# datatypevoid/babble

Measured on AMD Instinct MI355X. Metric: consensus-ordered events/sec at N=256 peers (1 GPU and 8-GPU batched sims), higher is better.
Workload: dtype int32

## Files before the change

### babble_amd/csrc/hgx_cts.hip

```cpp
#include <hip/hip_runtime.h>

#include <algorithm>
#include <climits>
#include <cstdint>

#include "hgx_device.h"
#include "hgx_kernels.h"

namespace hgx {

constexpr int kCpT = 8;
constexpr int kCpRing = 4;
constexpr int kCpMaxC = 4096;
constexpr int64_t kCtsRedo = (int64_t)0x8000000000000000ull;

struct CtsTileInfo {
    int32_t row[kCpT];
    int64_t ts[kCpT];
    int32_t tc, p0;
};

__device__ __forceinline__ void cp_lds_barrier() { asm volatile("s_waitcnt lgkmcnt(0)\n\ts_barrier" ::: "memory"); }
__device__ __forceinline__ void cp_order() { asm volatile("" ::: "memory"); }

template <int NPAD, typename CT>
__global__ void __launch_bounds__(256) k_cts_pipe(const int32_t* __restrict__ fu, const int32_t* __restrict__ rcnt,
                                                  const int32_t* __restrict__ p_rr, const int32_t* __restrict__ c_off,
                                                  const int32_t* __restrict__ c_base, const int32_t* __restrict__ WLAT, const CT* __restrict__ FDT,
                                                  const int64_t* __restrict__ p_ts, int64_t* __restrict__ p_cts, int C,
                                                  int n, int64_t Pcap, int c_lo, int c_cnt, int ntt) {
    constexpr int T = kCpT, LD = T + 1, NG = 256 / T, U = NPAD / NG, CPL = NPAD / 64;
    extern __shared__ __attribute__((aligned(16))) uint8_t dyn[];
    int32_t* kd = (int32_t*)dyn;
    int32_t* tp0 = kd + C;
    int32_t* trc = tp0 + c_cnt;
    uint32_t* vals = (uint32_t*)(dyn + ((4 * (C + 2 * c_cnt) + 15) & ~15));
    uint8_t* memb = (uint8_t*)(vals + 2 * NPAD * LD);
    __shared__ CtsTileInfo ring[kCpRing];
    __shared__ __attribute__((aligned(16))) uint32_t whist[4][256];

    const int t = threadIdx.x;
    for (int c = t; c < C; c += 256) kd[c] = c_off[c] - c_base[c];
    for (int c = t; c < c_cnt; c += 256) {
        tp0[c] = c_off[c_lo + c] + fu[c_lo + c];
        trc[c] = rcnt[c_lo + c];
    }
    __syncthreads();
    const int total = c_cnt * ntt;
    const int gstep = (int)gridDim.x;
    auto next_tile = [&](int u) -> int {
        for (; u < total; u += gstep) {
            const int ci = u % c_cnt, tt = u / c_cnt;
            if (tt * T < trc[ci]) break;
        }
        return __builtin_amdgcn_readfirstlane(min(u, total));
    };
    const int e = t & (T - 1), cg = t / T;
    int32_t l1_rr = -1;
    int64_t l1_ts = 0;
    bool l1_in = false;
    auto l1_issue = [&](int u) {
        const bool vu = u < total;
        const int ci = vu ? u % c_cnt : 0, tt = vu ? u / c_cnt : 0;
        l1_in = vu && tt * T + e < trc[ci];
        const int p = l1_in ? tp0[ci] + tt * T + e : 0;
        l1_rr = p_rr[p];
        l1_ts = p_ts[p];
    };
    auto l1_store = [&](int u, int slot) {
        const bool vu = u < total;
        const int ci = vu ? u % c_cnt : 0, tt = vu ? u / c_cnt : 0;
        int32_t rr_v = l1_in ? l1_rr : -1;
        int64_t ts_v = l1_ts;
        asm volatile("" : "+v"(rr_v), "+v"(ts_v));
        if (t < T) {
            ring[slot].row[t] = rr_v;
            ring[slot].ts[t] = ts_v;
            if (t == 0) {
                ring[slot].tc = c_lo + ci;
                ring[slot].p0 = tp0[ci] + tt * T;
            }
        }
    };
    int32_t l2_w[U];
    CT l2_fd[U];
    auto l2_issue = [&](int slot) {
        const int i = ring[slot].row[e];
        const int tc = ring[slot].tc, g = tc / n;
        const int p = ring[slot].p0 + e;
        const size_t fb = (size_t)max(i, 0) * C + (size_t)g * n;
        const size_t wrow = (fb + (tc - g * n)) * n;
#pragma unroll
        for (int u = 0; u < U; u++) {
            const int c = cg + NG * u;
            const bool in = i >= 0 && c < n;
            const int cc = in ? c : 0;
            l2_w[u] = WLAT[wrow + cc];
            l2_fd[u] = FDT[(size_t)cc * Pcap + (in ? p : 0)];
        }
    };
    int32_t idx[U];
    auto l2_finish = [&](int slot) {
        const int i = ring[slot].row[e];
        const int tc = ring[slot].tc, g = tc / n;
        const int j = ring[slot].p0 + e - kd[tc];
#pragma unroll
        for (int u = 0; u < U; u++) {
            const int c = cg + NG * u;
            const bool in = i >= 0 && c < n;
            const int cc = in ? c : 0;
            const int32_t k = kd[g * n + cc] + Coord<CT>::fd(l2_fd[u]);
            idx[u] = (in & (l2_w[u] >= j)) ? k : -1;
        }
    };

    int u0 = next_tile(blockIdx.x);
    if (u0 >= total) return;
    int u1 = next_tile(u0 + gstep);
    int u2 = next_tile(u1 + gstep);
    l1_issue(u0);
    l1_store(u0, 0);
    l1_issue(u1);
    l1_store(u1, 1);
    __syncthreads();
    l2_issue(0);
    l2_finish(0);
    const int lane = lane_id(), wave = t >> 6;
    int64_t x[U];
#pragma unroll
    for (int u = 0; u < U; u++) x[u] = p_ts[max(idx[u], 0)];
    cp_order();
    l2_issue(1);
    cp_order();
    l1_issue(u2);
    cp_order();

    for (int k = 0; u0 < total; k++) {
        const int s0 = k & (kCpRing - 1), s1 = (k + 1) & (kCpRing - 1), s2 = (k + 2) & (kCpRing - 1);
        {
            uint32_t* v = vals + (k & 1) * NPAD * LD;
            uint8_t* mb = memb + (k & 1) * NPAD * LD;
            const int64_t base = ring[s0].ts[e];
#pragma unroll
            for (int u = 0; u < U; u++) {
                const int c = cg + NG * u;
                const bool ok = idx[u] >= 0;
                const int64_t dlt = x[u] - base;
                const bool ov = ok && (dlt < INT32_MIN || dlt > INT32_MAX);
                v[c * LD + e] = (uint32_t)(int32_t)dlt ^ 0x80000000u;
                mb[c * LD + e] = (uint8_t)((ok ? 1 : 0) | (ov ? 2 : 0));
            }
        }
        l2_finish(s1);
        l1_store(u2, s2);
        cp_lds_barrier();
        const int u3 = next_tile(u2 + gstep);
#pragma unroll
        for (int u = 0; u < U; u++) x[u] = p_ts[max(idx[u], 0)];
        cp_order();
        l2_issue(s2);
        cp_order();
        l1_issue(u3);
        cp_order();
        {
            const uint32_t* v = vals + (k & 1) * NPAD * LD;
            const uint8_t* mb = memb + (k & 1) * NPAD * LD;
            for (int ev = wave; ev < T; ev += 4) {
                if (ring[s0].row[ev] < 0) continue;
                bool ok[CPL];
                uint32_t vv[CPL];
                int m = 0;
                bool any_ov = false;
#pragma unroll
                for (int q = 0; q < CPL; q++) {
                    const int c = lane + 64 * q;
                    const uint8_t b = mb[c * LD + ev];
                    ok[q] = (b & 1) != 0;
                    vv[q] = v[c * LD + ev];
                    m += __popcll(__ballot(ok[q]));
                    any_ov |= __ballot((b & 2) != 0) != 0;
                }
                int64_t res = kCtsRedo;
                if (!any_ov) {
                    const uint32_t sel = wave_select_kth32<CPL>(vv, ok, m / 2, whist[wave]);
                    res = ring[s0].ts[ev] + (int64_t)(int32_t)(sel ^ 0x80000000u);
                }
                if (lane == 0) p_cts[ring[s0].p0 + ev] = res;
            }
        }
        u0 = u1;
        u1 = u2;
        u2 = u3;
    }
}

template <int NPAD, typename CT>
__global__ void __launch_bounds__(256) k_cts_redo(const int32_t* __restrict__ fu, const int32_t* __restrict__ rcnt,
                                                  const int32_t* __restrict__ p_rr, const int32_t* __restrict__ c_off,
                                                  const int32_t* __restrict__ c_base, const int32_t* __restrict__ WLAT,
                                                  const CT* __restrict__ FDT, const int64_t* __restrict__ p_ts,
                                                  int64_t* __restrict__ p_cts, int C, int n, int64_t Pcap, int c_lo) {
    constexpr int CPL = NPAD / 64;
    __shared__ int32_t list[256];
    __shared__ int32_t cnt;
    __shared__ __attribute__((aligned(16))) uint32_t whist[4][256];
    const int gc = c_lo + blockIdx.y, g = gc / n;
    const int k = (int)blockIdx.x * 256 + threadIdx.x;
    if (threadIdx.x == 0) cnt = 0;
    __syncthreads();
    const int64_t p0 = (int64_t)c_off[gc] + fu[gc];
    if (k < rcnt[gc] && p_cts[p0 + k] == kCtsRedo) list[atomicAdd(&cnt, 1)] = k;
    __syncthreads();
    const int lane = lane_id(), wave = threadIdx.x >> 6;
    for (int q0 = wave; q0 < cnt; q0 += 4) {
        const int64_t p = p0 + list[q0];
        const int i = p_rr[p];
        const int j = c_base[gc] + (int)(p - c_off[gc]);
        const size_t row = ((size_t)i * C + gc) * n;
        uint64_t v[CPL];
        bool ok[CPL];
        int m = 0;
#pragma unroll
        for (int q = 0; q < CPL; q++) {
            const int c = lane + 64 * q;
            ok[q] = c < n && WLAT[row + c] >= j;
            int64_t x = 0;
            if (ok[q]) {
                const int ch = g * n + c;
                x = p_ts[c_off[ch] - c_base[ch] + Coord<CT>::fd(FDT[(size_t)c * Pcap + p])];
            }
            v[q] = (uint64_t)x ^ 0x8000000000000000ull;
            m += __popcll(__ballot(ok[q]));
        }
        const int64_t res = (int64_t)(wave_select_kth<CPL>(v, ok, m / 2, whist[wave]) ^ 0x8000000000000000ull);
        if (lane == 0) p_cts[p] = res;
    }
}

template <int NPAD, typename CT>
static bool cts_pipe_launch(hipStream_t s, const DevArrays& a, int c_lo, int c_cnt, int C, int n, int64_t P,
                            int max_cnt) {
    constexpr int LD = kCpT + 1;
    const size_t lds = (((size_t)4 * C + (size_t)8 * c_cnt + 15) & ~(size_t)15) + (size_t)2 * NPAD * LD * 5;
    const void* f = (const void*)k_cts_pipe<NPAD, CT>;
    static int dev_cus[64] = {0};
    int dev = 0;
    if (hipGetDevice(&dev) != hipSuccess || dev < 0 || dev >= 64) return false;
    if (ensure_lds_limit(f, lds) != hipSuccess) return false;
    if (dev_cus[dev] == 0) {
        int cus = 0;
        if (hipDeviceGetAttribute(&cus, hipDeviceAttributeMultiprocessorCount, dev) != hipSuccess || cus <= 0)
            return false;
        dev_cus[dev] = cus;
    }
    int per_cu = 0;
    if (blocks_per_cu(f, 256, lds, &per_cu) != hipSuccess || per_cu < 1) return false;
    const int ntt = (max_cnt + kCpT - 1) / kCpT;
    const int64_t tiles = (int64_t)c_cnt * ntt;
    if (tiles <= 0) return true;
    if (tiles > 0x7FFFFFFF - (int64_t)dev_cus[dev] * per_cu) return false;
    const unsigned grid = (unsigned)std::min<int64_t>(tiles, (int64_t)dev_cus[dev] * per_cu);
    hipLaunchKernelGGL((k_cts_pipe<NPAD, CT>), dim3(grid), dim3(256), lds, s, a.fu, a.rcnt, a.p_rr, a.c_off, a.c_base,
                       a.WLAT, (const CT*)a.FDT, a.p_ts, a.p_cts, C, n, P, c_lo, c_cnt, ntt);
    hipLaunchKernelGGL((k_cts_redo<NPAD, CT>), dim3((max_cnt + 255) / 256, c_cnt), dim3(256), 0, s, a.fu, a.rcnt, a.p_rr,
                       a.c_off, a.c_base, a.WLAT, (const CT*)a.FDT, a.p_ts, a.p_cts, C, n, P, c_lo);
    return true;
}

template <typename CT>
static bool launch_cts_pipe_t(hipStream_t s, const DevArrays& a, int c_lo, int c_cnt, int C, int n, int64_t P,
                              int max_cnt) {
    if (n <= 64) return cts_pipe_launch<64, CT>(s, a, c_lo, c_cnt, C, n, P, max_cnt);
    if (n <= 128) return cts_pipe_launch<128, CT>(s, a, c_lo, c_cnt, C, n, P, max_cnt);
    if (n <= 256) return cts_pipe_launch<256, CT>(s, a, c_lo, c_cnt, C, n, P, max_cnt);
    return cts_pipe_launch<512, CT>(s, a, c_lo, c_cnt, C, n, P, max_cnt);
}

bool cts_pipe_ok(int n, int C) { return n > 32 && n <= 512 && C <= kCpMaxC; }

bool launch_cts_pipe(hipStream_t s, const DevArrays& a, int c_lo, int c_cnt, int C, int n, int64_t P, int max_cnt) {
    if (max_cnt <= 0 || c_cnt <= 0) return true;
    if (!cts_pipe_ok(n, C)) return false;
    return a.compact ? launch_cts_pipe_t<uint16_t>(s, a, c_lo, c_cnt, C, n, P, max_cnt)
                     : launch_cts_pipe_t<int32_t>(s, a, c_lo, c_cnt, C, n, P, max_cnt);
}

constexpr int kRowKMax = 8;
constexpr int kRowTP = 64;
constexpr int kRowD = 16;
constexpr int row_waves(int npad) { return npad >= 128 ? 8 : 4; }

template <int NPAD, typename CT, int TP, int DREQ, int NW>
__global__ void __launch_bounds__(64 * NW) k_cts_row(const int32_t* __restrict__ fu, const int32_t* __restrict__ rcnt,
                                                 const int32_t* __restrict__ p_rr, const int32_t* __restrict__ c_off,
                                                 const int32_t* __restrict__ c_base, const int32_t* __restrict__ WLAT,
                                                 const CT* __restrict__ FDT, const int64_t* __restrict__ p_ts,
                                                 int64_t* __restrict__ p_cts, int C, int n, int64_t Pcap, int c_lo,
                                                 int c_cnt, int R, int K) {
    static_assert(TP == 64, "k_cts_row: a wave's lanes are the block's events");
    constexpr int LD = TP + 1;
    constexpr int CPL = NPAD / 64;
    constexpr int CW = NPAD / NW;
    constexpr int NI = CW;
    constexpr int D = DREQ < NI ? DREQ : NI;
    constexpr int NB = NI / D;
    constexpr int MB = NPAD / 8;
    static_assert(NI % D == 0 && NI % 8 == 0 && NI <= 64, "k_cts_row: batches and membership bytes");
    constexpr int RG = 64 * NW / NPAD;
    constexpr int KL = kRowKMax / RG;
    static_assert(RG >= 1 && kRowKMax % RG == 0, "k_cts_row: staging loads");
    extern __shared__ __attribute__((aligned(16))) uint32_t vals[];
    int32_t* wl = (int32_t*)(vals + NPAD * LD);
    __shared__ uint8_t mem[TP][MB];
    __shared__ int32_t e_row[TP];
    __shared__ int64_t e_ts[TP];
    __shared__ int32_t e_ovf[TP];
    __shared__ uint32_t s_min[NW];
    const int cl = (int)(blockIdx.x % (unsigned)c_cnt), tt = (int)(blockIdx.x / (unsigned)c_cnt);
    const int tc = c_lo + cl;
    const int f0 = fu[tc], co = c_off[tc];
    const int64_t q0 = (int64_t)co + f0, pend = q0 + rcnt[tc];
    const int64_t ps = (int64_t)co + (f0 & ~31) + (int64_t)tt * TP;
    if ((ps > q0 ? ps : q0) >= pend) return;
    const int lane = lane_id(), wave = __builtin_amdgcn_readfirstlane((int)(threadIdx.x >> 6));
    const int e = lane;
    const int64_t p = ps + e;
    const bool ev = p >= q0 && p < pend;
    const int64_t pl = ev ? p : (ps > q0 ? ps : q0);
    const int i = p_rr[pl];
    const int64_t base = p_ts[pl];
    const int g = tc / n, gb = g * n;
    const int j = c_base[tc] + (int)(pl - co);
    const bool evi = ev && i >= 0;
    const int wc0 = wave * CW;
    uint32_t* whist = vals + NPAD * LD + 256 * wave;
    auto chain = [&](int k) { const int c = wc0 + k; return c < n ? c : 0; };
    auto load_fd = [&](int b, CT (&fd)[D]) {
#pragma unroll
        for (int u = 0; u < D; u++) fd[u] = FDT[(size_t)chain(b * D + u) * Pcap + pl];
    };
    CT fd[2][D];
    load_fd(0, fd[0]);
    const int kc = wc0 + lane < n && lane < CW ? wc0 + lane : 0;
    const int32_t kdv = c_off[gb + kc] - c_base[gb + kc];
    const uint32_t wmin = wave_reduce_min_u32(evi ? (uint32_t)i : 0x7fffffffu);
    if (lane == 0) s_min[wave] = wmin;
    if (threadIdx.x < TP) {
        e_row[e] = evi ? i : -1;
        e_ts[e] = base;
        e_ovf[e] = 0;
    }
    cp_lds_barrier();
    uint32_t bmin = s_min[0];
#pragma unroll
    for (int w = 1; w < NW; w++) bmin = min(bmin, s_min[w]);
    const int imin = bmin == 0x7fffffffu ? 0 : (int)bmin;
    int32_t st[KL];
    const int sw = (int)threadIdx.x % NPAD, srow = (int)threadIdx.x / NPAD;
#pragma unroll
    for (int q = 0; q < KL; q++)
        st[q] = WLAT[((size_t)min(imin + min(q * RG + srow, K - 1), R - 1) * C + tc) * n + min(sw, n - 1)];
    int64_t x[2][D];
    auto gather = [&](int b, const CT (&f)[D], int64_t (&xo)[D]) {
#pragma unroll
        for (int u = 0; u < D; u++) {
            const int k = b * D + u;
            const int32_t kd = __builtin_amdgcn_readlane(kdv, k);
            const int32_t fv = Coord<CT>::fd(f[u]);
            xo[u] = p_ts[fv != kMaxI32 ? kd + fv : 0];
        }
    };
    uint64_t ovm = 0;
    if (NB > 1) load_fd(1, fd[1]);
    cp_order();
    gather(0, fd[0], x[0]);
    cp_order();
#pragma unroll
    for (int b = 0; b < NB; b++) {
        if (b + 2 < NB) load_fd(b + 2, fd[b & 1]);
        cp_order();
        if (b + 1 < NB) gather(b + 1, fd[(b + 1) & 1], x[(b + 1) & 1]);
        cp_order();
#pragma unroll
        for (int u = 0; u < D; u++) {
            const int k = b * D + u;
            const int64_t dlt = x[b & 1][u] - base;
            ovm |= (uint64_t)(dlt < INT32_MIN || dlt > INT32_MAX) << k;
            vals[(wc0 + k) * LD + e] = (uint32_t)(int32_t)dlt ^ 0x80000000u;
        }
        cp_order();
    }
    const int WS = n + 1;
#pragma unroll
    for (int q = 0; q < KL; q++)
        if (q * RG + srow < K && sw < n) wl[(q * RG + srow) * WS + sw] = st[q];
    __syncthreads();
    {
        uint64_t okm = 0;
        if (!evi || i - imin < K) {
            const int32_t* row = wl + (evi ? i - imin : 0) * WS;
#pragma unroll
            for (int k = 0; k < NI; k++) okm |= (uint64_t)(row[chain(k)] >= j) << k;
        } else {
            const int32_t* __restrict__ row = WLAT + ((size_t)i * C + tc) * n;
#pragma unroll
            for (int k = 0; k < NI; k++) okm |= (uint64_t)(row[chain(k)] >= j) << k;
        }
        const int live = n - wc0;
        if (live < NI) okm &= live > 0 ? ((uint64_t)1 << live) - 1 : 0;
        if (!evi) okm = 0;
#pragma unroll
        for (int q = 0; q < NI / 8; q++) mem[e][wc0 / 8 + q] = (uint8_t)(okm >> (8 * q));
        if (ovm & okm) e_ovf[e] = 1;
    }
    __syncthreads();
    for (int e2 = wave; e2 < TP; e2 += NW) {
        if (e_row[e2] < 0) continue;
        bool ok[CPL];
        int m = 0;
#pragma unroll
        for (int q = 0; q < CPL; q++) {
            const int c = lane + 64 * q;
            ok[q] = (mem[e2][c >> 3] >> (c & 7)) & 1u;
            m += __popcll(__builtin_amdgcn_ballot_w64(ok[q]));
        }
        int64_t res;
        if (!e_ovf[e2]) {
            uint32_t v[CPL];
#pragma unroll
            for (int q = 0; q < CPL; q++) v[q] = vals[(lane + 64 * q) * LD + e2];
            const uint32_t u = wave_select_kth32_top<CPL>(v, ok, m / 2, whist);
            res = e_ts[e2] + (int64_t)(int32_t)(u ^ 0x80000000u);
        } else {
            uint64_t v[CPL];
#pragma unroll
            for (int q = 0; q < CPL; q++) {
                const int c = lane + 64 * q;
                int64_t x = 0;
                if (ok[q]) x = p_ts[c_off[gb + c] - c_base[gb + c] + Coord<CT>::fd(FDT[(size_t)c * Pcap + ps + e2])];
                v[q] = (uint64_t)x ^ 0x8000000000000000ull;
            }
            res = (int64_t)(wave_select_kth<CPL>(v, ok, m / 2, whist) ^ 0x8000000000000000ull);
        }
        if (lane == 0) p_cts[ps + e2] = res;
    }
}

template <int NPAD, typename CT>
static bool cts_row_launch(hipStream_t s, const DevArrays& a, int c_lo, int c_cnt, int C, int n, int64_t P,
                           int max_cnt, int R, int k_rows) {
    constexpr int TP = kRowTP, NW = row_waves(NPAD);
    constexpr size_t kStatic = (size_t)TP * (NPAD / 8) + (size_t)TP * 16 + 4 * NW;
    const size_t fixed = (size_t)NPAD * (TP + 1) * 4, row = (size_t)(n + 1) * 4;
    const int room = (int)(((size_t)79 * 1024 - kStatic - fixed) / row);
    const int K = k_rows > 0 ? std::min(k_rows, kRowKMax) : std::max(1, std::min(room, kRowKMax));
    const size_t lds = fixed + std::max((size_t)K * row, (size_t)NW * 1024);
    const void* f = (const void*)k_cts_row<NPAD, CT, TP, kRowD, NW>;
    if (ensure_lds_limit(f, lds) != hipSuccess) return false;
    const int64_t blocks = (int64_t)c_cnt * ((max_cnt + 31 + TP - 1) / TP);
    if (blocks > 0x7FFFFFFF) return false;
    hipLaunchKernelGGL((k_cts_row<NPAD, CT, TP, kRowD, NW>), dim3((unsigned)blocks), dim3(64 * NW), lds, s, a.fu, a.rcnt, a.p_rr,
                       a.c_off, a.c_base, a.WLAT, (const CT*)a.FDT, a.p_ts, a.p_cts, C, n, P, c_lo, c_cnt, R, K);
    return true;
}

template <typename CT>
static bool launch_cts_row_t(hipStream_t s, const DevArrays& a, int c_lo, int c_cnt, int C, int n, int64_t P,
                             int max_cnt, int R, int k_rows) {
    if (n <= 64) return cts_row_launch<64, CT>(s, a, c_lo, c_cnt, C, n, P, max_cnt, R, k_rows);
    if (n <= 128) return cts_row_launch<128, CT>(s, a, c_lo, c_cnt, C, n, P, max_cnt, R, k_rows);
    return cts_row_launch<256, CT>(s, a, c_lo, c_cnt, C, n, P, max_cnt, R, k_rows);
}

bool cts_row_ok(int n) { return n > 32 && n <= 256; }
int cts_row_tile() { return kRowTP; }

bool launch_cts_row(hipStream_t s, const DevArrays& a, int c_lo, int c_cnt, int C, int n, int64_t P, int max_cnt,
                    int R, int k_rows) {
    if (max_cnt <= 0 || c_cnt <= 0) return true;
    if (!cts_row_ok(n) || R <= 0) return false;
    return a.compact ? launch_cts_row_t<uint16_t>(s, a, c_lo, c_cnt, C, n, P, max_cnt, R, k_rows)
                     : launch_cts_row_t<int32_t>(s, a, c_lo, c_cnt, C, n, P, max_cnt, R, k_rows);
}

}
```

### babble_amd/csrc/hgx_device.h

```cpp
#pragma once

#include <hip/hip_runtime.h>

#include <cstdint>

namespace hgx {

__device__ __forceinline__ int lane_id() { return (int)(threadIdx.x & 63); }

__device__ __forceinline__ uint32_t block_excl_scan256(uint32_t v, uint32_t* sh, uint32_t* total) {
    const int lane = lane_id(), wave = threadIdx.x >> 6;
    uint32_t x = v;
    for (int o = 1; o < 64; o <<= 1) {
        const uint32_t y = __shfl_up(x, o);
        if (lane >= o) x += y;
    }
    if (lane == 63) sh[wave] = x;
    __syncthreads();
    uint32_t wbase = 0;
    for (int w = 0; w < wave; w++) wbase += sh[w];
    *total = sh[0] + sh[1] + sh[2] + sh[3];
    __syncthreads();
    return wbase + x - v;
}

template <int HD>
__device__ __forceinline__ uint32_t swar_ge_count(const uint32_t (&v)[HD], const uint32_t (&nf)[HD]) {
    uint32_t c = 0;
    if constexpr (HD % 2 == 0) {
#pragma unroll
        for (int i = 0; i < HD / 2; i++) {
            const uint64_t s = ((((uint64_t)v[2 * i + 1]) << 32) | v[2 * i]) + ((((uint64_t)nf[2 * i + 1]) << 32) | nf[2 * i]);
            c = __builtin_popcount((uint32_t)s & 0x80808080u) + c;
            asm volatile("" : "+v"(c));
            c = __builtin_popcount((uint32_t)(s >> 32) & 0x80808080u) + c;
            asm volatile("" : "+v"(c));
        }
    } else {
#pragma unroll
        for (int d = 0; d < HD; d++) c += __builtin_popcount((v[d] + nf[d]) & 0x80808080u);
    }
    return c;
}
__device__ __forceinline__ uint32_t swar_nf(uint32_t fd7) { return 0x80808080u - fd7; }

__device__ __forceinline__ uint64_t group_mask(int gs, int grp) {
    return (gs >= 64) ? ~0ull : (((1ull << gs) - 1ull) << (gs * grp));
}

template <typename CT>
struct Coord;
template <>
struct Coord<int32_t> {
    static constexpr int32_t kLaNone = -1;
    __device__ __forceinline__ static int32_t la(int32_t v) { return v; }
    __device__ __forceinline__ static int32_t enc_la(int32_t v) { return v; }
    __device__ __forceinline__ static int32_t fd(int32_t v) { return v; }
    __device__ __forceinline__ static int32_t enc_fd(int32_t v) { return v; }
};
template <>
struct Coord<uint16_t> {
    static constexpr int32_t kLaNone = 0;
    __device__ __forceinline__ static int32_t la(uint32_t v) { return (int32_t)v - 1; }
    __device__ __forceinline__ static uint16_t enc_la(int32_t v) { return (uint16_t)(v + 1); }
    __device__ __forceinline__ static int32_t fd(uint32_t v) { return v == 0xFFFFu ? 2147483647 : (int32_t)v; }
    __device__ __forceinline__ static uint16_t enc_fd(int32_t v) { return v >= 0xFFFF ? (uint16_t)0xFFFF : (uint16_t)v; }
};

__device__ __forceinline__ void wave_lds_fence() {
    __builtin_amdgcn_fence(__ATOMIC_SEQ_CST, "wavefront");
    __builtin_amdgcn_wave_barrier();
}

__device__ __forceinline__ uint64_t wave_min_u64(uint64_t x) {
    for (int o = 32; o >= 1; o >>= 1) {
        const uint64_t y = __shfl_xor(x, o);
        x = y < x ? y : x;
    }
    return x;
}

__device__ __forceinline__ uint64_t wave_max_u64(uint64_t x) {
    for (int o = 32; o >= 1; o >>= 1) {
        const uint64_t y = __shfl_xor(x, o);
        x = y > x ? y : x;
    }
    return x;
}

template <int CPL>
__device__ uint64_t wave_select_kth(const uint64_t (&v)[CPL], const bool (&ok)[CPL], int K,
                                    uint32_t* __restrict__ hist) {
    const int lane = lane_id();
    uint64_t lo = ~0ull, hi = 0;
#pragma unroll
    for (int q = 0; q < CPL; q++)
        if (ok[q]) { lo = v[q] < lo ? v[q] : lo; hi = v[q] > hi ? v[q] : hi; }
    lo = wave_min_u64(lo);
    hi = wave_max_u64(hi);
    bool act[CPL];
#pragma unroll
    for (int q = 0; q < CPL; q++) act[q] = ok[q];
    uint64_t base = lo;
    uint64_t range = hi - lo;
    int k = K;
    while (range != 0) {
        int bits = 64 - __clzll((long long)range);
        const int shift = bits > 8 ? bits - 8 : 0;
#pragma unroll
        for (int t = 0; t < 4; t++) hist[lane * 4 + t] = 0;
        wave_lds_fence();
#pragma unroll
        for (int q = 0; q < CPL; q++)
            if (act[q]) atomicAdd(&hist[(uint32_t)((v[q] - base) >> shift)], 1u);
        wave_lds_fence();
        uint32_t h[4], s = 0;
#pragma unroll
        for (int t = 0; t < 4; t++) { h[t] = hist[lane * 4 + t]; s += h[t]; }
        uint32_t incl = s;
        for (int o = 1; o < 64; o <<= 1) {
            const uint32_t y = __shfl_up(incl, o);
            if (lane >= o) incl += y;
        }
        const uint32_t excl = incl - s;
        int bucket = -1;
        uint32_t below = 0;
        if ((uint32_t)k >= excl && (uint32_t)k < incl) {
            uint32_t acc = excl;
#pragma unroll
            for (int t = 0; t < 4; t++) {
                if (bucket < 0 && (uint32_t)k < acc + h[t]) { bucket = lane * 4 + t; below = acc; }
                acc += h[t];
            }
        }
        const uint64_t bm = __ballot(bucket >= 0);
        const int src = __ffsll((unsigned long long)bm) - 1;
        bucket = __shfl(bucket, src);
        below = __shfl(below, src);
        wave_lds_fence();
        k -= (int)below;
        const uint64_t nb = base + ((uint64_t)bucket << shift);
#pragma unroll
        for (int q = 0; q < CPL; q++) act[q] = act[q] && ((v[q] - base) >> shift) == (uint64_t)bucket;
        if (shift == 0) return nb;
        const uint64_t top = nb + ((1ull << shift) - 1);
        base = nb;
        range = (top < hi ? top : hi) - nb;
        uint64_t alo = ~0ull, ahi = 0;
#pragma unroll
        for (int q = 0; q < CPL; q++)
            if (act[q]) { alo = v[q] < alo ? v[q] : alo; ahi = v[q] > ahi ? v[q] : ahi; }
        alo = wave_min_u64(alo);
        ahi = wave_max_u64(ahi);
        base = alo;
        range = ahi - alo;
    }
    return base;
}

#define HGX_DPP_SCAN(x, id, OP)                                                                  \
    do {                                                                                         \
        x = OP(x, (uint32_t)__builtin_amdgcn_update_dpp((int)(id), (int)(x), 0x111, 0xf, 0xf, false)); \
        x = OP(x, (uint32_t)__builtin_amdgcn_update_dpp((int)(id), (int)(x), 0x112, 0xf, 0xf, false)); \
        x = OP(x, (uint32_t)__builtin_amdgcn_update_dpp((int)(id), (int)(x), 0x114, 0xf, 0xf, false)); \
        x = OP(x, (uint32_t)__builtin_amdgcn_update_dpp((int)(id), (int)(x), 0x118, 0xf, 0xf, false)); \
        x = OP(x, (uint32_t)__builtin_amdgcn_update_dpp((int)(id), (int)(x), 0x142, 0xa, 0xf, false)); \
        x = OP(x, (uint32_t)__builtin_amdgcn_update_dpp((int)(id), (int)(x), 0x143, 0xc, 0xf, false)); \
    } while (0)
#define HGX_OP_ADD(a, b) ((a) + (b))
#define HGX_OP_MIN(a, b) min((a), (b))
#define HGX_OP_MAX(a, b) max((a), (b))

__device__ __forceinline__ uint32_t wave_scan_add_u32(uint32_t x) { HGX_DPP_SCAN(x, 0u, HGX_OP_ADD); return x; }
__device__ __forceinline__ uint32_t wave_reduce_min_u32(uint32_t x) {
    HGX_DPP_SCAN(x, 0xffffffffu, HGX_OP_MIN);
    return (uint32_t)__builtin_amdgcn_readlane((int)x, 63);
}
__device__ __forceinline__ uint32_t wave_reduce_max_u32(uint32_t x) {
    HGX_DPP_SCAN(x, 0u, HGX_OP_MAX);
    return (uint32_t)__builtin_amdgcn_readlane((int)x, 63);
}

template <int CPL>
__device__ uint32_t wave_select_kth32(const uint32_t (&v)[CPL], const bool (&ok)[CPL], int K,
                                      uint32_t* __restrict__ hist) {
    const int lane = lane_id();
    uint32_t lo = 0xffffffffu, hi = 0;
#pragma unroll
    for (int q = 0; q < CPL; q++)
        if (ok[q]) { lo = min(lo, v[q]); hi = max(hi, v[q]); }
    lo = wave_reduce_min_u32(lo);
    hi = wave_reduce_max_u32(hi);
    const uint32_t range = hi - lo;
    if (range == 0) return lo;
    const int bits = 32 - __clz((int)range);
    uint32_t d[CPL];
    bool act[CPL];
#pragma unroll
    for (int q = 0; q < CPL; q++) { d[q] = v[q] - lo; act[q] = ok[q]; }
    uint4* __restrict__ h4 = (uint4*)hist;
    uint32_t prefix = 0;
    uint32_t k = (uint32_t)K;
    for (int shift = ((bits - 1) / 8) * 8; shift >= 0; shift -= 8) {
        h4[lane] = make_uint4(0u, 0u, 0u, 0u);
        wave_lds_fence();
#pragma unroll
        for (int q = 0; q < CPL; q++)
            if (act[q]) atomicAdd(&hist[(d[q] >> shift) & 255u], 1u);
        wave_lds_fence();
        const uint4 h = h4[lane];
        const uint32_t sum = h.x + h.y + h.z + h.w;
        const uint32_t incl = wave_scan_add_u32(sum);
        const uint32_t excl = incl - sum;
        const uint32_t a1 = excl + h.x, a2 = a1 + h.y, a3 = a2 + h.z;
        const int bt = (k < a1) ? 0 : (k < a2) ? 1 : (k < a3) ? 2 : 3;
        const uint32_t below = (k < a1) ? excl : (k < a2) ? a1 : (k < a3) ? a2 : a3;
        const uint64_t bm = __ballot(k >= excl && k < incl);
        const int src = (int)__builtin_ctzll(bm);
        const uint32_t bucket = (uint32_t)__builtin_amdgcn_readlane(lane * 4 + bt, src);
        k -= (uint32_t)__builtin_amdgcn_readlane((int)below, src);
        wave_lds_fence();
        prefix |= bucket << shift;
#pragma unroll
        for (int q = 0; q < CPL; q++) act[q] = act[q] && ((d[q] >> shift) & 255u) == bucket;
    }
    return lo + prefix;
}

template <int CPL>
__device__ __forceinline__ uint32_t wave_select_kth32_top(const uint32_t (&v)[CPL], const bool (&ok)[CPL], int K,
                                                          uint32_t* __restrict__ hist) {
    constexpr int DB = 6;
    const int lane = lane_id();
    uint32_t lo = 0xffffffffu, hi = 0;
#pragma unroll
    for (int q = 0; q < CPL; q++)
        if (ok[q]) { lo = min(lo, v[q]); hi = max(hi, v[q]); }
    lo = wave_reduce_min_u32(lo);
    hi = wave_reduce_max_u32(hi);
    if (hi <= lo) return lo;
    int top = 32 - __clz((int)(hi - lo));
    uint32_t d[CPL], inc[CPL];
#pragma unroll
    for (int q = 0; q < CPL; q++) { d[q] = v[q] - lo; inc[q] = ok[q] ? 1u : 0u; }
    uint32_t prefix = 0, k = (uint32_t)K;
#pragma unroll 1
    for (int pass = 0; pass < (32 + DB - 1) / DB; pass++) {
        const int shift = top > DB ? top - DB : 0;
        uint32_t dig[CPL];
#pragma unroll
        for (int q = 0; q < CPL; q++) dig[q] = __builtin_amdgcn_ubfe(d[q], (uint32_t)shift, (uint32_t)(top - shift));
        hist[lane] = 0;
        wave_lds_fence();
#pragma unroll
        for (int q = 0; q < CPL; q++) atomicAdd(&hist[dig[q]], inc[q]);
        wave_lds_fence();
        const uint32_t h = hist[lane];
        wave_lds_fence();
        const uint32_t incl = wave_scan_add_u32(h);
        const uint32_t excl = incl - h;
        const uint64_t bm = __builtin_amdgcn_ballot_w64(k >= excl) & __builtin_amdgcn_ballot_w64(k < incl);
        const int bucket = bm ? (int)__builtin_ctzll(bm) : 0;
        k -= (uint32_t)__builtin_amdgcn_readlane((int)excl, bucket);
        const uint32_t cnt = (uint32_t)__builtin_amdgcn_readlane((int)h, bucket);
        prefix |= (uint32_t)bucket << shift;
        if (shift == 0) break;
#pragma unroll
        for (int q = 0; q < CPL; q++) inc[q] = dig[q] == (uint32_t)bucket ? inc[q] : 0u;
        if (cnt == 1u) {
            uint32_t r = lo + prefix;
#pragma unroll
            for (int q = 0; q < CPL; q++) {
                const uint64_t b = __builtin_amdgcn_ballot_w64(inc[q] != 0u);
                if (b) r = (uint32_t)__builtin_amdgcn_readlane((int)v[q], (int)__builtin_ctzll(b));
            }
            return r;
        }
        top = shift;
    }
    return lo + prefix;
}

template <int CPL>
__device__ uint32_t wave_select_kth32_bisect(const uint32_t (&v)[CPL], const bool (&ok)[CPL], int K) {
    uint32_t lo = 0xffffffffu, hi = 0;
#pragma unroll
    for (int q = 0; q < CPL; q++)
        if (ok[q]) { lo = min(lo, v[q]); hi = max(hi, v[q]); }
    lo = wave_reduce_min_u32(lo);
    hi = wave_reduce_max_u32(hi);
    uint32_t a = 0, b = hi - lo;
    uint32_t d[CPL];
#pragma unroll
    for (int q = 0; q < CPL; q++) d[q] = ok[q] ? v[q] - lo : 0xffffffffu;
    while (a < b) {
        const uint32_t mid = a + ((b - a) >> 1);
        int cnt = 0;
#pragma unroll
        for (int q = 0; q < CPL; q++) cnt += __popcll(__ballot(d[q] <= mid));
        if (cnt > K) b = mid;
        else a = mid + 1;
    }
    return lo + a;
}

}
```

Before: 274.8 million.

## Select per-event median with 8-lane groups instead of whole waves

Replaces the per-event whole-wave radix selection with 8-lane DPP groups, so each wave processes 8 events at once. Membership is packed into transposed 32-bit words via LDS atomicOr, and a new group8 radix-select runs its histogram in the event's own column of the vals buffer. Overflow events still fall back to the wave-wide 64-bit selection. The new path adds LDS atomics and more complex control flow, and it restricts NI to at most 32.

```diff
diff --git a/babble_amd/csrc/hgx_cts.hip b/babble_amd/csrc/hgx_cts.hip
--- a/babble_amd/csrc/hgx_cts.hip
+++ b/babble_amd/csrc/hgx_cts.hip
@@ -304,14 +304,14 @@
     constexpr int NI = CW;
     constexpr int D = DREQ < NI ? DREQ : NI;
     constexpr int NB = NI / D;
-    constexpr int MB = NPAD / 8;
-    static_assert(NI % D == 0 && NI % 8 == 0 && NI <= 64, "k_cts_row: batches and membership bytes");
+    constexpr int VPL = NPAD / 8;
+    static_assert(NI % D == 0 && NI % 8 == 0 && NI <= 32 && 8 % NW == 0, "k_cts_row: batches, membership words, groups");
     constexpr int RG = 64 * NW / NPAD;
     constexpr int KL = kRowKMax / RG;
     static_assert(RG >= 1 && kRowKMax % RG == 0, "k_cts_row: staging loads");
     extern __shared__ __attribute__((aligned(16))) uint32_t vals[];
     int32_t* wl = (int32_t*)(vals + NPAD * LD);
-    __shared__ uint8_t mem[TP][MB];
+    __shared__ uint32_t memw[8 * LD];
     __shared__ int32_t e_row[TP];
     __shared__ int64_t e_ts[TP];
     __shared__ int32_t e_ovf[TP];
@@ -350,6 +350,7 @@
         e_ts[e] = base;
         e_ovf[e] = 0;
     }
+    for (int w = (int)threadIdx.x; w < 8 * LD; w += 64 * NW) memw[w] = 0;
     cp_lds_barrier();
     uint32_t bmin = s_min[0];
 #pragma unroll
@@ -409,40 +410,46 @@
         const int live = n - wc0;
         if (live < NI) okm &= live > 0 ? ((uint64_t)1 << live) - 1 : 0;
         if (!evi) okm = 0;
-#pragma unroll
-        for (int q = 0; q < NI / 8; q++) mem[e][wc0 / 8 + q] = (uint8_t)(okm >> (8 * q));
+        const uint32_t ok32 = (uint32_t)okm;
+#pragma unroll
+        for (int l = 0; l < 8; l++)
+            atomicOr(&memw[l * LD + e], ((((ok32 >> l) & 0x01010101u) * 0x10204080u) >> 28) << (wc0 / 8));
         if (ovm & okm) e_ovf[e] = 1;
     }
     __syncthreads();
-    for (int e2 = wave; e2 < TP; e2 += NW) {
-        if (e_row[e2] < 0) continue;
-        bool ok[CPL];
-        int m = 0;
-#pragma unroll
-        for (int q = 0; q < CPL; q++) {
-            const int c = lane + 64 * q;
-            ok[q] = (mem[e2][c >> 3] >> (c & 7)) & 1u;
-            m += __popcll(__builtin_amdgcn_ballot_w64(ok[q]));
-        }
-        int64_t res;
-        if (!e_ovf[e2]) {
-            uint32_t v[CPL];
-#pragma unroll
-            for (int q = 0; q < CPL; q++) v[q] = vals[(lane + 64 * q) * LD + e2];
-            const uint32_t u = wave_select_kth32_top<CPL>(v, ok, m / 2, whist);
-            res = e_ts[e2] + (int64_t)(int32_t)(u ^ 0x80000000u);
-        } else {
+    const int gs = lane >> 3, gl = lane & 7;
+    for (int grp = 0; grp < 8 / NW; grp++) {
+        const int vw = wave + NW * grp, e2 = vw + 8 * gs;
+        const bool has = e_row[e2] >= 0, wide = e_ovf[e2] != 0;
+        if (!__builtin_amdgcn_ballot_w64(has)) continue;
+        const bool part = has && !wide;
+        if (__builtin_amdgcn_ballot_w64(part)) {
+            uint32_t* hcol = vals + e2;
+            const uint32_t member = part ? memw[gl * LD + e2] : 0u;
+            uint32_t v[VPL];
+#pragma unroll
+            for (int q = 0; q < VPL; q++) v[q] = hcol[(gl + 8 * q) * LD];
+            const uint32_t u = group8_select_kth32_top<VPL, LD>(v, member, hcol, whist + 32 * gs, gl);
+            if (part && gl == 0) p_cts[ps + e2] = e_ts[e2] + (int64_t)(int32_t)(u ^ 0x80000000u);
+        }
+        for (uint64_t todo = __builtin_amdgcn_ballot_w64(has && wide) & 0x0101010101010101ull; todo; todo &= todo - 1) {
+            const int e3 = vw + (int)__builtin_ctzll(todo);
+            const uint32_t mw = memw[gl * LD + e3];
+            bool ok[CPL];
             uint64_t v[CPL];
+            int m = 0;
 #pragma unroll
             for (int q = 0; q < CPL; q++) {
                 const int c = lane + 64 * q;
+                ok[q] = (mw >> (gs + 8 * q)) & 1u;
+                m += __popcll(__builtin_amdgcn_ballot_w64(ok[q]));
                 int64_t x = 0;
-                if (ok[q]) x = p_ts[c_off[gb + c] - c_base[gb + c] + Coord<CT>::fd(FDT[(size_t)c * Pcap + ps + e2])];
+                if (ok[q]) x = p_ts[c_off[gb + c] - c_base[gb + c] + Coord<CT>::fd(FDT[(size_t)c * Pcap + ps + e3])];
                 v[q] = (uint64_t)x ^ 0x8000000000000000ull;
             }
-            res = (int64_t)(wave_select_kth<CPL>(v, ok, m / 2, whist) ^ 0x8000000000000000ull);
-        }
-        if (lane == 0) p_cts[ps + e2] = res;
+            const int64_t res = (int64_t)(wave_select_kth<CPL>(v, ok, m / 2, whist) ^ 0x8000000000000000ull);
+            if (lane == 0) p_cts[ps + e3] = res;
+        }
     }
 }
 
@@ -450,7 +457,7 @@
 static bool cts_row_launch(hipStream_t s, const DevArrays& a, int c_lo, int c_cnt, int C, int n, int64_t P,
                            int max_cnt, int R, int k_rows) {
     constexpr int TP = kRowTP, NW = row_waves(NPAD);
-    constexpr size_t kStatic = (size_t)TP * (NPAD / 8) + (size_t)TP * 16 + 4 * NW;
+    constexpr size_t kStatic = (size_t)8 * (TP + 1) * 4 + (size_t)TP * 16 + 4 * NW;
     const size_t fixed = (size_t)NPAD * (TP + 1) * 4, row = (size_t)(n + 1) * 4;
     const int room = (int)(((size_t)79 * 1024 - kStatic - fixed) / row);
     const int K = k_rows > 0 ? std::min(k_rows, kRowKMax) : std::max(1, std::min(room, kRowKMax));
diff --git a/babble_amd/csrc/hgx_device.h b/babble_amd/csrc/hgx_device.h
--- a/babble_amd/csrc/hgx_device.h
+++ b/babble_amd/csrc/hgx_device.h
@@ -281,6 +281,148 @@
     return lo + prefix;
 }
 
+template <int CTRL, int BANK = 0xf>
+__device__ __forceinline__ uint32_t dpp_mov0(uint32_t x) {
+    return (uint32_t)__builtin_amdgcn_update_dpp(0, (int)x, CTRL, 0xf, BANK, false);
+}
+#define HGX_DPP_GROUP8(x, OP)                    \
+    do {                                         \
+        x = OP(x, dpp_mov0<0xB1>(x));            \
+        x = OP(x, dpp_mov0<0x4E>(x));            \
+        x = OP(x, dpp_mov0<0x141>(x));           \
+    } while (0)
+#define HGX_OP_OR(a, b) ((a) | (b))
+__device__ __forceinline__ uint32_t group8_add_u32(uint32_t x) { HGX_DPP_GROUP8(x, HGX_OP_ADD); return x; }
+__device__ __forceinline__ uint32_t group8_or_u32(uint32_t x) { HGX_DPP_GROUP8(x, HGX_OP_OR); return x; }
+__device__ __forceinline__ uint32_t group8_min_u32(uint32_t x) { HGX_DPP_GROUP8(x, HGX_OP_MIN); return x; }
+__device__ __forceinline__ uint32_t group8_max_u32(uint32_t x) { HGX_DPP_GROUP8(x, HGX_OP_MAX); return x; }
+__device__ __forceinline__ uint32_t group8_scan_add_u32(uint32_t x, int l) {
+    const uint32_t y1 = dpp_mov0<0x111>(x);
+    x += l >= 1 ? y1 : 0u;
+    const uint32_t y2 = dpp_mov0<0x112>(x);
+    x += l >= 2 ? y2 : 0u;
+    x += dpp_mov0<0x114, 0xA>(x);
+    return x;
+}
+
+
+struct Group8Sel {
+    uint32_t lo, res, prefix, k;
+    int top;
+    bool live;
+};
+
+template <int NV, int LD>
+__device__ __forceinline__ uint32_t group8_select_pass(const uint32_t (&d)[NV], uint32_t& act, Group8Sel& s,
+                                                       uint32_t* hcol, int l) {
+    constexpr int DB = 6;
+    const int shift = s.top > DB ? s.top - DB : 0;
+    const uint32_t width = (uint32_t)(s.top - shift);
+    auto bin = [&](uint32_t b) -> uint32_t* { return (uint32_t*)((char*)hcol + __umul24(b, (uint32_t)(LD * 4))); };
+#pragma unroll
+    for (int t = 0; t < 8; t++) hcol[(l + 8 * t) * LD] = 0;
+    wave_lds_fence();
+#pragma unroll
+    for (int q = 0; q < NV; q++) atomicAdd(bin(__builtin_amdgcn_ubfe(d[q], (uint32_t)shift, width)), (act >> q) & 1u);
+    wave_lds_fence();
+    uint32_t h[8];
+#pragma unroll
+    for (int t = 0; t < 8; t++) h[t] = hcol[(l + 8 * t) * LD];
+    wave_lds_fence();
+    uint32_t acc = 0, below = 0, hsel = 0, tsel = 0;
+#pragma unroll
+    for (int t = 0; t < 8; t++) {
+        const bool c = s.k >= acc;
+        below = c ? acc : below;
+        hsel = c ? h[t] : hsel;
+        tsel = c ? (uint32_t)t : tsel;
+        acc += group8_add_u32(h[t]);
+    }
+    const uint32_t k1 = s.k - below;
+    const uint32_t incl = group8_scan_add_u32(hsel, l), excl = incl - hsel;
+    const bool own = k1 >= excl && k1 < incl;
+    const uint32_t pk = group8_or_u32(own ? (tsel * 8 + (uint32_t)l) | excl << 6 | hsel << 16 : 0u);
+    const uint32_t bucket = pk & 63u, cnt = pk >> 16;
+    s.k = k1 - ((pk >> 6) & 1023u);
+    s.prefix |= bucket << shift;
+    const bool last = shift == 0, one = cnt == 1u;
+    if (__builtin_amdgcn_ballot_w64(s.live && !last)) {
+        uint32_t keep = 0;
+#pragma unroll
+        for (int q = 0; q < NV; q++) keep |= __builtin_amdgcn_ubfe(d[q], (uint32_t)shift, width) == bucket ? 1u << q : 0u;
+        act &= keep;
+    }
+    if (__builtin_amdgcn_ballot_w64(s.live && !last && one)) {
+        uint32_t w = 0xffffffffu;
+#pragma unroll
+        for (int q = 0; q < NV; q++) w = min(w, d[q] | ~(uint32_t)__builtin_amdgcn_sbfe((int)act, q, 1));
+        w = group8_min_u32(w);
+        s.res = s.live && !last && one ? s.lo + w : s.res;
+    }
+    s.res = s.live && last ? s.lo + s.prefix : s.res;
+    s.live = s.live && !last && !one;
+    act = s.live ? act : 0u;
+    s.top = shift;
+    return cnt;
+}
+
+template <int VPL, int LD>
+__device__ __forceinline__ uint32_t group8_select_kth32_top(uint32_t (&v)[VPL], uint32_t member, uint32_t* hcol,
+                                                            uint32_t* list, int l) {
+    constexpr int DB = 6, PASSES = (32 + DB - 1) / DB, CAP = 32, LV = CAP / 8;
+    uint32_t lo = 0xffffffffu, hi = 0;
+#pragma unroll
+    for (int q = 0; q < VPL; q++) {
+        const uint32_t in = (uint32_t)__builtin_amdgcn_sbfe((int)member, q, 1);
+        lo = min(lo, v[q] | ~in);
+        hi = max(hi, v[q] & in);
+    }
+    lo = group8_min_u32(lo);
+    hi = group8_max_u32(hi);
+    const uint32_t m = group8_add_u32((uint32_t)__popc(member));
+    Group8Sel s;
+    s.lo = lo;
+    s.res = lo;
+    s.prefix = 0;
+    s.k = m >> 1;
+    s.live = hi > lo;
+    s.top = s.live ? 32 - __clz((int)(hi - lo)) : 0;
+#pragma unroll
+    for (int q = 0; q < VPL; q++) v[q] -= lo;
+    uint32_t act = s.live ? member : 0u;
+    if (!__builtin_amdgcn_ballot_w64(s.live)) return s.res;
+    const uint32_t cnt = group8_select_pass<VPL, LD>(v, act, s, hcol, l);
+    if (!__builtin_amdgcn_ballot_w64(s.live)) return s.res;
+    if (VPL > LV && !__builtin_amdgcn_ballot_w64(s.live && cnt > (uint32_t)CAP)) {
+        const uint32_t mine = (uint32_t)__popc(act);
+        uint32_t pos = group8_scan_add_u32(mine, l) - mine;
+#pragma unroll
+        for (int q = 0; q < VPL; q++)
+            if ((act >> q) & 1u) list[pos++ & (CAP - 1)] = v[q];
+        wave_lds_fence();
+        uint32_t w[LV], wact = 0;
+#pragma unroll
+        for (int j = 0; j < LV; j++) {
+            w[j] = list[l + 8 * j];
+            wact |= (uint32_t)(l + 8 * j) < cnt ? 1u << j : 0u;
+        }
+        wact = s.live ? wact : 0u;
+        wave_lds_fence();
+#pragma unroll 1
+        for (int pass = 1; pass < PASSES; pass++) {
+            group8_select_pass<LV, LD>(w, wact, s, hcol, l);
+            if (!__builtin_amdgcn_ballot_w64(s.live)) break;
+        }
+    } else {
+#pragma unroll 1
+        for (int pass = 1; pass < PASSES; pass++) {
+            group8_select_pass<VPL, LD>(v, act, s, hcol, l);
+            if (!__builtin_amdgcn_ballot_w64(s.live)) break;
+        }
+    }
+    return s.res;
+}
+
 template <int CPL>
 __device__ uint32_t wave_select_kth32_bisect(const uint32_t (&v)[CPL], const bool (&ok)[CPL], int K) {
     uint32_t lo = 0xffffffffu, hi = 0;
```

Measured after the change: 280.9 million, median of 6. 2.2% higher.
